# Zehong-Ma/OVMR

Measured on AMD Instinct MI355X. Metric: images/sec ViT-B/16 encode+fusion, 1k-class×16-shot, 1/2/4/8 MI355X, higher is better.
Workload: dtype f16; 1 GPU; OVMR classifier generation + fusion inference, ViT-B/16, 1000 classes x 16 shots (16000 exemplar images, batch 775) + 4096 query images (batch 256), n_ctx 2, tau 10; parallelism=class/query sharding over 1 rank(s); all-gather rows + all-reduce counters, preset=metric, gemm_variant=8, attn_variant=3, ln_fold=1, gelu_exact=0, stream_text=1, encoder_reserve_images=775, encoder_chunk_images=775, output_dir=tmpfs scratch (/dev/shm)

## Files before the change

### ovmr_amd/csrc/common.h

```cpp
#pragma once
#include <hip/hip_runtime.h>
#include <stdint.h>

typedef _Float16 half_t;
typedef _Float16 half2_t __attribute__((ext_vector_type(2)));
typedef _Float16 half4_t __attribute__((ext_vector_type(4)));
typedef _Float16 half8_t __attribute__((ext_vector_type(8)));
typedef float float4_t __attribute__((ext_vector_type(4)));
typedef float float2_t __attribute__((ext_vector_type(2)));

#define OVMR_WAVE 64
#define OVMR_MAX_DEVICES 64

enum {
    EPI_NONE = 0,
    EPI_BIAS = 1,
    EPI_BIAS_QGELU = 2,
    EPI_BIAS_RES = 3,
    EPI_PATCH = 4,
    EPI_SCALE = 5,
    EPI_LN_BIAS = 6,
    EPI_LN_BIAS_QGELU = 7,
    EPI_SCALE_ARGMAX = 8,
};

struct GemmArgs {
    const void* A; int lda;
    const void* W; int ldw;
    void* C; int ldc;
    const void* bias;
    const void* res; int ldres;
    const void* pos;
    int M, N, K;
    int epi;
    int rows_in, rows_out;
    float scale;
    int n_group;
    const float* ln_stats; int ln_slots;
    int ln_stride;
    const float* ln_g; const float* ln_b;
    float* stats_out;
    int nt_store;
    float* argmax_out;
    int gelu_mode;
    int im2col_R;
};

__device__ __forceinline__ float quick_gelu_h(float u) {
    half_t t = (half_t)(1.702f * u);
    half_t s = (half_t)__builtin_amdgcn_rcpf(1.0f + __builtin_amdgcn_exp2f(-1.4426950408889634f * (float)t));
    return (float)(half_t)(u * (float)s);
}

__device__ __forceinline__ half4_t quick_gelu_h4(half4_t u) {
    half4_t t;
    float4_t e;
#pragma unroll
    for (int k = 0; k < 4; ++k) {
        t[k] = (half_t)(1.702f * (float)u[k]);
        e[k] = __builtin_amdgcn_exp2f(fminf(__builtin_fmaf((float)t[k], -1.4426950408889634f, 0.0f), 30.0f));
    }
    const float2_t p = (float2_t){e[0], e[2]} + 1.0f, q = (float2_t){e[1], e[3]} + 1.0f;
    const float2_t pq = p * q;
    const float R = __builtin_amdgcn_rcpf(pq[0] * pq[1]);
    const float2_t rr = (float2_t){pq[1], pq[0]} * R;
// ... 46 lines not shown
```

### ovmr_amd/csrc/gemm_f16.hip

```cpp
#include "gemm_epi.h"
#include "gemm_route.h"

namespace {

constexpr int BK = 64;

template <int EPI>
__global__ __launch_bounds__(256) void gemm_f16_t128(GemmArgs a) {
    extern __shared__ __attribute__((aligned(16))) char smem[];
    half_t* sA = (half_t*)smem;
    half_t* sB = sA + 2 * 128 * BK;

    const int tid = threadIdx.x, lane = tid & 63, wave = tid >> 6;
    const int wm = wave >> 1, wn = wave & 1;
    const int tiles_n = (a.N + 127) >> 7;
    const int tm = blockIdx.x / tiles_n, tn = blockIdx.x - tm * tiles_n;
    const int m0 = tm << 7, n0 = tn << 7;

    const half_t* A = (const half_t*)a.A;
    const half_t* W = (const half_t*)a.W;

    const int lc = tid & 7, lr = tid >> 3;
    const int sw = ((lc ^ (lr & 7)) << 3);
    const half_t* ga[4];
// ... 81 lines not shown
        HIP_CHECK_RET(hipFuncSetAttribute((const void*)gemm_f16_t128<EPI>, hipFuncAttributeMaxDynamicSharedMemorySize, (int)lds));
        attr_set[dev] = true;
    }
    hipLaunchKernelGGL(gemm_f16_t128<EPI>, dim3(tiles), dim3(256), lds, s, a);
    return (int)hipGetLastError();
}

bool one_round_of_s64(int M, int N) { return (long)((M + 63) / 64) * ((N + 63) / 64) <= 256; }
bool aligned16(const void* p) { return ((uintptr_t)p & 15) == 0; }

void plan_tile(const GemmArgs& a, bool ping_pong, GemmPlan& p) {
    const int tiles_n = (a.N + 255) / 256;
    const double t256 = (double)((a.M + 255) / 256) * tiles_n, t128 = (double)((a.M + 127) / 128) * tiles_n;
    auto rounds = [](double t) { return ceil(t / 256.0); };
    auto eff = [&](double t) { return t / (rounds(t) * 256.0); };
    const bool big = ping_pong ? rounds(t256) <= 0.74 * rounds(t128) : t256 >= 64 && eff(t256) + 0.08 >= eff(t128);
    p.tile_rows = big ? 256 : 128;
    const int tiles = (int)(big ? t256 : t128);
    const bool res = a.epi == EPI_BIAS_RES, lnf = a.epi == EPI_LN_BIAS || a.epi == EPI_LN_BIAS_QGELU;
    p.loop = ping_pong && big ? LOOP_PINGPONG : (lnf || (res && a.K >= 2048)) ? LOOP_BOUNDARY : LOOP_DOUBLE;
    p.a_nt = res && tiles_n <= 4 && tiles >= 512;
    p.nt_store = !res && a.epi != EPI_SCALE_ARGMAX && (size_t)a.M * a.N * 2 >= ((size_t)48 << 20);
    p.n_group = p.loop == LOOP_PINGPONG && tiles_n >= 8 ? 4 : tiles_n;
}

}

bool gemm_f16_latency_bound(int variant, int M, int N) { return variant == 8 && one_round_of_s64(M, N); }
int gemm_f16_pinned_variant(int variant, int M, int N) { return variant != 8 ? variant : one_round_of_s64(M, N) ? 9 : 7; }

GemmPlan gemm_f16_route(const GemmArgs& a, int variant) {
    GemmPlan p = {};
    auto run = [&p](int kernel, int rc = 0) { p.kernel = kernel; p.rc = rc; return p; };
    auto none = [&run](int rc) { return run(GEMM_NONE, rc); };
    const bool lnf = a.epi == EPI_LN_BIAS || a.epi == EPI_LN_BIAS_QGELU, res = a.epi == EPI_BIAS_RES, argmax = a.epi == EPI_SCALE_ARGMAX;
    if (a.epi == EPI_BIAS_QGELU || a.epi == EPI_LN_BIAS_QGELU) p.gelu_mode = variant >= 100 ? variant / 100 : a.gelu_mode;
    if (variant >= 100) variant %= 100;
    if (a.M <= 0 || a.N <= 0) return none(0);
    if (a.K <= 0 || (a.K % BK) != 0 || (a.lda & 7) || (a.ldw & 7)) return none(-2);
    const bool tile_only = a.im2col_R || argmax || lnf || a.stats_out;
    if (!tile_only && (variant == 9 || gemm_f16_latency_bound(variant, a.M, a.N)) && (a.K % 128) == 0 && aligned16(a.A) && aligned16(a.W) && a.epi != EPI_PATCH &&
        a.epi >= EPI_NONE && a.epi <= EPI_SCALE) {
        const int steps = a.K >> 7, tiles = ((a.M + 63) >> 6) * ((a.N + 63) >> 6);
        p.depth = steps % 4 == 0 && tiles <= 256 ? 4 : steps % 3 == 0 ? 3 : steps % 2 == 0 ? 2 : 1;
        p.groups = steps / p.depth;
        return run(GEMM_S64);
// ... 1 lines not shown
    const bool takes = a.M >= 256 && a.N >= 128 && (long)a.M * a.lda * 2 < 0x7fffffffL && (long)a.N * a.ldw * 2 < 0x7fffffffL &&
                       (argmax ? a.argmax_out != nullptr
                               : !(a.N & 7) && !(a.ldc & 7) && aligned16(a.C) && (!res || (!(a.ldres & 7) && aligned16(a.res))));
    if ((tile_only || variant >= 1) && takes) {
        if (a.im2col_R) {
            const int G = a.im2col_R >> 4;
            if (a.epi != EPI_PATCH || a.K != 768 || (a.im2col_R & 15) || a.rows_in != G * G || !aligned16(a.A) ||
                (long)((a.M + a.rows_in - 1) / a.rows_in) * 3 * a.im2col_R * a.im2col_R * 2 >= 0x7fffffffL)
                return none(-2);
        }
        if (lnf && ((a.N & 63) || !a.ln_stats || a.ln_slots < 1 || !a.ln_g || !a.ln_b)) return none(-2);
        if (a.stats_out && (!res || (a.N & 255))) return none(-2);
        const int loop = (variant == 0 || variant == 7 || variant == 9) ? 8 : variant;
        if (loop != 6 && loop != 8) return none(-5);
        if (a.epi < EPI_NONE || a.epi > EPI_SCALE_ARGMAX) return none(-3);
        plan_tile(a, loop == 8 && (a.K % 128) == 0, p);
        return run(GEMM_TILE);
    }
    if (tile_only) return none(-4);
    if (a.epi < EPI_NONE || a.epi > EPI_SCALE) return none(-3);
    return run(GEMM_T128);
}

extern "C" int ovmr_debug_gemm_route(int variant, int M, int N, int K, int epi, int ldc, int ldres, int stats, int im2col, int* out) {
    static float operand[4];
    alignas(16) static char base[16];
    GemmArgs a = {};
    a.M = M; a.N = N; a.K = a.lda = a.ldw = K; a.epi = epi; a.ldc = ldc; a.ldres = ldres;
    a.A = a.W = a.res = base; a.C = base;
    a.ln_stats = a.ln_g = a.ln_b = operand; a.ln_slots = 1; a.argmax_out = operand; a.stats_out = stats ? operand : nullptr;
    a.im2col_R = im2col; a.rows_in = (im2col >> 4) * (im2col >> 4); a.rows_out = a.rows_in + 1;
    static_assert(sizeof(GemmPlan) == 10 * sizeof(int), "");
    *(GemmPlan*)out = gemm_f16_route(a, variant);
    return 0;
}

int launch_gemm_f16(const GemmArgs& a_in, int variant, hipStream_t s) {
    const GemmPlan p = gemm_f16_route(a_in, variant);
    GemmArgs a = a_in;
    a.n_group = p.n_group;
    a.gelu_mode = p.gelu_mode;
    switch (p.kernel) {
        case GEMM_T128:
#define X(E) if (a.epi == E) return launch_t128<E>(a, s);
            X(EPI_NONE) X(EPI_BIAS) X(EPI_BIAS_QGELU) X(EPI_BIAS_RES) X(EPI_PATCH) X(EPI_SCALE)
#undef X
            return -3;
        case GEMM_S64: return launch_gemm_f16_small(a, p, s);
        case GEMM_TILE: return launch_gemm_f16_v5(a, p, s);
    }
    return p.rc;
}
```

### ovmr_amd/csrc/gemm_f16_v5.hip

```cpp
#include "gemm_route.h"

namespace {

constexpr int BK5 = 64, BN5 = 256;
typedef const __attribute__((address_space(1))) void* gptr_t;
typedef __attribute__((address_space(3))) void* lptr_t;

template <int CTRL>
__device__ __forceinline__ float dpp_f32(float v) {
    return __builtin_bit_cast(float, __builtin_amdgcn_update_dpp(0, __builtin_bit_cast(int, v), CTRL, 0xF, 0xF, true));
}

constexpr int OPT_A_NT = 1;
constexpr int OPT_BOUNDARY = 4;
constexpr int OPT_PINGPONG = 16;
constexpr int OPT_NT_STORE = 512;
constexpr int OPT_GELU_F32 = 2048;
template <int EPI, int MT, int OPT>
__global__ __launch_bounds__(512) void gemm_f16_v5_kernel(GemmArgs a, int tiles_m, int tiles_n) {
    constexpr int BM = MT * 32;
    constexpr int A_BYTES = BM * 128, STAGE = (BM + BN5) * 128;
    constexpr int AJ = BM / 64;
    constexpr bool NT = OPT & OPT_NT_STORE;
    constexpr int EP = 128;
    constexpr bool GFAST = (OPT & OPT_GELU_F32) != 0;
    constexpr bool LNF = EPI == EPI_LN_BIAS || EPI == EPI_LN_BIAS_QGELU;
    constexpr bool HAS_BIAS = EPI == EPI_BIAS || EPI == EPI_BIAS_QGELU || EPI == EPI_BIAS_RES;
    extern __shared__ __attribute__((aligned(16))) char smem[];
    float* col_c = (float*)(smem + 2 * STAGE);
    float* row_c = col_c + 2 * BN5;

    const int tid = threadIdx.x, lane = tid & 63;
    const int wave = __builtin_amdgcn_readfirstlane(tid >> 6);
    const int wm = wave >> 2, wn = wave & 3;

    const int nwg = tiles_m * tiles_n;
    int bid = blockIdx.x;
    {
        const int xcd = bid & 7, idx = bid >> 3, q = nwg >> 3, r = nwg & 7;
        bid = (xcd < r ? xcd * (q + 1) : r * (q + 1) + (xcd - r) * q) + idx;
    }
    int tm, tn;
    {
        const int G = a.n_group > 0 ? a.n_group : tiles_n;
        const int full = tiles_n / G, per = tiles_m * G;
        const int g = bid / per;
        if (g < full) {
            const int r = bid - g * per;
            tm = r / G;
            tn = g * G + (r - tm * G);
        } else {
            const int Gl = tiles_n - full * G, r = bid - full * per;
            tm = r / Gl;
            tn = full * G + (r - tm * Gl);
        }
    }
    const int m0 = tm * BM, n0 = tn * BN5;

    const int nk = a.K / BK5;
    const half_t* A = (const half_t*)a.A;
    const half_t* W = (const half_t*)a.W;

    const int srow = lane >> 3, slot = lane & 7;
    const int schunk = (slot ^ srow) * 8;
    unsigned oa[AJ], ob[4];
    auto src_off = [&](int row, int ld) -> unsigned { return (unsigned)(((long)row * ld + schunk) * 2); };
    const int imR = (EPI == EPI_PATCH) ? a.im2col_R : 0;
    auto a_off = [&](int row) -> unsigned {
        if (EPI == EPI_PATCH && imR) {
            const int G = imR >> 4, r = min(row, a.M - 1), b = r / a.rows_in, p = r - b * a.rows_in, gy = p / G, gx = p - gy * G;
            const int c8 = schunk >> 3;
            return (unsigned)(2 * (((long)b * 3 * imR + gy * 16 + (c8 >> 1)) * imR + gx * 16 + (c8 & 1) * 8));
        }
        return src_off(min(row, a.M - 1), a.lda);
    };
    auto a_tile = [&](int kt) -> const char* {
        if (EPI == EPI_PATCH && imR) return (const char*)A + 2 * ((long)(kt >> 2) * imR * imR + (kt & 3) * 4 * imR);
        return (const char*)A + (long)kt * 128;
    };
#pragma unroll
// ... 9 lines not shown
    const int ldsA_w = wave * (BM / 8) * 128;
    const int ldsB_w = A_BYTES + wave * 32 * 128;

    auto stage = [&](int buf, int kt) {
        char* base = smem + buf * STAGE;
#pragma unroll
        for (int j = 0; j < AJ; ++j)
            __builtin_amdgcn_global_load_lds((gptr_t)(a_tile(kt) + oa[j]), (lptr_t)(base + ldsA_w + j * 1024), 16, 0, (OPT & OPT_A_NT) ? 2 : 0);
#pragma unroll
        for (int j = 0; j < 4; ++j)
            __builtin_amdgcn_global_load_lds((gptr_t)((const char*)W + ob[j] + (long)kt * 128), (lptr_t)(base + ldsB_w + j * 1024), 16, 0, 0);
    };

    float4_t acc[MT][4];
#pragma unroll
    for (int i = 0; i < MT; ++i)
#pragma unroll
        for (int j = 0; j < 4; ++j) acc[i][j] = (float4_t){0.f, 0.f, 0.f, 0.f};

    const int fr = lane & 15, fg = lane >> 4;
    const int a_row_off = (wm * (BM / 2) + fr) * 128;
    const int b_row_off = A_BYTES + (wn * 64 + fr) * 128;
    const int ch0 = ((fg) ^ (fr & 7)) << 4, ch1 = ((4 + fg) ^ (fr & 7)) << 4;

    constexpr bool PH8 = (OPT & OPT_PINGPONG) != 0 && MT == 8;
    if (!PH8) stage(0, 0);

    if (PH8) {
    } else if (tid < BN5) {
        const int n = n0 + tid;
        float c0 = 0.f, c1 = 0.f;
        if (n < a.N) {
            if (HAS_BIAS) c0 = (float)((const half_t*)a.bias)[n];
            if (LNF) { c0 = a.ln_g[n]; c1 = a.ln_b[n]; }
        }
        col_c[tid] = c0;
        col_c[BN5 + tid] = c1;
    } else if (LNF && tid - BN5 < BM) {
        const int r = tid - BN5;
        const float2_t* sp = (const float2_t*)a.ln_stats + (long)min(m0 + r, a.M - 1) * (a.ln_stride ? a.ln_stride : a.ln_slots);
        float su = 0.f, sq = 0.f;
        for (int sl = 0; sl < a.ln_slots; ++sl) { const float2_t p = sp[sl]; su += p[0]; sq += p[1]; }
        const float inv_k = 1.0f / (float)a.K;
        const float mean = su * inv_k;
        const float rstd = 1.0f / sqrtf(fmaxf(sq * inv_k - mean * mean, 0.f) + 1e-5f);
        row_c[r] = rstd;
        row_c[BM + r] = -rstd * mean;
    }

    if constexpr (PH8) {
    constexpr int SLOT = 16384, KBUF = 4 * SLOT;
    enum { hB0 = 0, hA0 = 1, hB1 = 2, hA1 = 3 };
    unsigned sa8[2][2], sb8[2][2];
#pragma unroll
    for (int hf = 0; hf < 2; ++hf)
#pragma unroll
        for (int j = 0; j < 2; ++j) {
            const int lr = wave * 16 + j * 8 + srow;
            const int ra = m0 + (lr >> 6) * 128 + hf * 64 + (lr & 63);
            const int rb = n0 + (lr >> 5) * 64 + hf * 32 + (lr & 31);
            sa8[hf][j] = a_off(ra);
            sb8[hf][j] = src_off(min(rb, a.N - 1), a.ldw);
        }
    const unsigned smem_lds = __builtin_amdgcn_readfirstlane((unsigned)(uintptr_t)(lptr_t)smem);
    const unsigned wave_lds = (unsigned)__builtin_amdgcn_readfirstlane(wave * 2048);
    auto stage_half = [&](int buf, int which, int kt) {
        const int hf = which >> 1;
        const char* ak = a_tile(kt);
        const char* wk = (const char*)W + (long)kt * 128;
#pragma unroll
        for (int j = 0; j < 2; ++j) {
            const unsigned dst = smem_lds + (unsigned)(buf * KBUF + which * SLOT + j * 1024) + wave_lds;
            if (which & 1) {
                if constexpr ((OPT & OPT_A_NT) != 0) asm volatile("s_mov_b32 m0, %2\n\ts_nop 0\n\tglobal_load_lds_dwordx4 %0, %1 nt" :: "v"(sa8[hf][j]), "s"(ak), "s"(dst) : "memory", "m0");
                else asm volatile("s_mov_b32 m0, %2\n\ts_nop 0\n\tglobal_load_lds_dwordx4 %0, %1" :: "v"(sa8[hf][j]), "s"(ak), "s"(dst) : "memory", "m0");
            } else {
                asm volatile("s_mov_b32 m0, %2\n\ts_nop 0\n\tglobal_load_lds_dwordx4 %0, %1" :: "v"(sb8[hf][j]), "s"(wk), "s"(dst) : "memory", "m0");
            }
        }
    };
    const int a_lane = (wm * 64 + fr) * 128, b_lane = (wn * 32 + fr) * 128;
    half8_t fa[4][2], fb0[2][2], fb1[2][2];
    auto read_a = [&](const char* buf, int hf) {
#pragma unroll
        for (int ii = 0; ii < 4; ++ii) {
            fa[ii][0] = *(const half8_t*)(buf + (1 + 2 * hf) * SLOT + a_lane + ii * 2048 + ch0);
// ... 2 lines not shown
    };
    auto read_b = [&](const char* buf, int g, half8_t (&fb)[2][2]) {
#pragma unroll
        for (int jj = 0; jj < 2; ++jj) {
            fb[jj][0] = *(const half8_t*)(buf + 2 * g * SLOT + b_lane + jj * 2048 + ch0);
            fb[jj][1] = *(const half8_t*)(buf + 2 * g * SLOT + b_lane + jj * 2048 + ch1);
        }
    };
    auto quadrant = [&](int hf, int g, half8_t (&fb)[2][2]) {
        __builtin_amdgcn_s_setprio(1);
#pragma unroll
        for (int st = 0; st < 2; ++st)
#pragma unroll
            for (int ii = 0; ii < 4; ++ii)
#pragma unroll
                for (int jj = 0; jj < 2; ++jj)
                    acc[hf * 4 + ii][g * 2 + jj] = __builtin_amdgcn_mfma_f32_16x16x32_f16(fb[jj][st], fa[ii][st], acc[hf * 4 + ii][g * 2 + jj], 0, 0, 0);
        __builtin_amdgcn_s_setprio(0);
    };
#define OVMR_PH_END()                                                     \
    __builtin_amdgcn_sched_barrier(0);                                    \
    __builtin_amdgcn_s_barrier();                                         \
    __builtin_amdgcn_sched_barrier(0);
    stage_half(0, hB0, 0); stage_half(0, hA0, 0); stage_half(0, hB1, 0); stage_half(0, hA1, 0);
    if (tid < BN5) {
        const int n = n0 + tid;
        float c0 = 0.f, c1 = 0.f;
        if (n < a.N) {
            if (HAS_BIAS) c0 = (float)((const half_t*)a.bias)[n];
            if (LNF) { c0 = a.ln_g[n]; c1 = a.ln_b[n]; }
        }
        col_c[tid] = c0;
        col_c[BN5 + tid] = c1;
    } else if (LNF && tid - BN5 < BM) {
        const int r = tid - BN5;
        const float2_t* sp = (const float2_t*)a.ln_stats + (long)min(m0 + r, a.M - 1) * (a.ln_stride ? a.ln_stride : a.ln_slots);
        float su = 0.f, sq = 0.f;
        for (int sl = 0; sl < a.ln_slots; ++sl) { const float2_t p = sp[sl]; su += p[0]; sq += p[1]; }
        const float inv_k = 1.0f / (float)a.K;
        const float mean = su * inv_k;
        const float rstd = 1.0f / sqrtf(fmaxf(sq * inv_k - mean * mean, 0.f) + 1e-5f);
        row_c[r] = rstd;
        row_c[BM + r] = -rstd * mean;
    }
    __builtin_amdgcn_sched_barrier(0);
    stage_half(1, hB0, 1); stage_half(1, hA0, 1);
    asm volatile("s_waitcnt vmcnt(4)" ::: "memory");
    asm volatile("s_waitcnt lgkmcnt(0)" ::: "memory");
    __builtin_amdgcn_s_barrier();
    __builtin_amdgcn_sched_barrier(0);
    if (wm == 1) __builtin_amdgcn_s_barrier();
    __builtin_amdgcn_sched_barrier(0);
    const char* const bufE = smem;
    const char* const bufO = smem + KBUF;
#define OVMR_P4_MID()                                                     \
    __builtin_amdgcn_sched_barrier(0);                                    \
    asm volatile("s_waitcnt lgkmcnt(0)" ::: "memory");                    \
    __builtin_amdgcn_s_barrier();                                         \
    __builtin_amdgcn_sched_barrier(0);
    for (int kt = 0; kt < nk; kt += 2) {
        const bool more = kt + 2 < nk;
        read_b(bufE, 0, fb0);
        read_a(bufE, 0);
        read_b(bufE, 1, fb1);
        __builtin_amdgcn_sched_barrier(0);
        stage_half(1, hB1, kt + 1); stage_half(1, hA1, kt + 1);
        OVMR_P4_MID()
        quadrant(0, 0, fb0);
        quadrant(0, 1, fb1);
// ... 10 lines not shown
        OVMR_PH_END()
        read_b(bufO, 0, fb0);
        read_a(bufO, 0);
        read_b(bufO, 1, fb1);
        __builtin_amdgcn_sched_barrier(0);
        if (more) { stage_half(0, hB1, kt + 2); stage_half(0, hA1, kt + 2); }
        OVMR_P4_MID()
        quadrant(0, 0, fb0);
        quadrant(0, 1, fb1);
        OVMR_PH_END()
        read_a(bufO, 1);
        __builtin_amdgcn_sched_barrier(0);
        if (more) { stage_half(1, hB0, kt + 3); stage_half(1, hA0, kt + 3); }
        __builtin_amdgcn_sched_barrier(0);
        if (more) asm volatile("s_waitcnt vmcnt(4)" ::: "memory");
        OVMR_P4_MID()
        quadrant(1, 1, fb1);
        quadrant(1, 0, fb0);
        OVMR_PH_END()
    }
#undef OVMR_P4_MID
    if (wm == 0) __builtin_amdgcn_s_barrier();
    __builtin_amdgcn_sched_barrier(0);
#undef OVMR_PH_END
    } else
    if (OPT & OPT_BOUNDARY) {
    constexpr int D = 2, R = D + 2;
    static_assert((2 * MT) % R == 0 && D <= MT, "");
    half8_t fb[2][4], fa[R];
    auto first_reads = [&](const char* buf) {
#pragma unroll
        for (int t = 0; t < 4; ++t) fb[0][t] = *(const half8_t*)(buf + b_row_off + t * 2048 + ch0);
#pragma unroll
        for (int t = 0; t < D; ++t) fa[t] = *(const half8_t*)(buf + a_row_off + (t % MT) * 2048 + (t / MT ? ch1 : ch0));
    };
    asm volatile("s_waitcnt vmcnt(0)" ::: "memory");
    asm volatile("s_waitcnt lgkmcnt(0)" ::: "memory");
    __builtin_amdgcn_s_barrier();
    __builtin_amdgcn_sched_barrier(0);
    first_reads(smem);
    __builtin_amdgcn_sched_barrier(0);
    if (nk > 1) stage(1, 1);
    __builtin_amdgcn_sched_barrier(0);
    for (int kt = 0; kt < nk; ++kt) {
        const char* cur = smem + (kt & 1) * STAGE;
#pragma unroll
// ... 109 lines not shown
                int* d = arg_lds + ((wm * (BM / 2) + i * 16 + fr) * 4 + wn) * 2;
                d[0] = __float_as_int(bv);
                d[1] = bc;
            }
        }
        __syncthreads();
        if (tid < BM && m0 + tid < a.M) {
            float bv = __int_as_float(arg_lds[tid * 8]);
            int bc = arg_lds[tid * 8 + 1];
#pragma unroll
            for (int w = 1; w < 4; ++w) {
                const float v = __int_as_float(arg_lds[tid * 8 + 2 * w]);
                const int vc = arg_lds[tid * 8 + 2 * w + 1];
                if (v > bv || (v == bv && vc < bc)) { bv = v; bc = vc; }
            }
            int* dst = (int*)a.argmax_out + ((long)(m0 + tid) * tiles_n + tn) * 2;
            dst[0] = __float_as_int(bv);
            dst[1] = bc;
        }
        return;
    }
    char* et = smem + wave * (64 * EP);
    const int er = lane >> 3, ec = (lane & 7) * 8;
    const int fsw = ((fr & 7) << 1) | (fr >> 3);
    int wr_off[4];
#pragma unroll
    for (int j = 0; j < 4; ++j) wr_off[j] = fr * EP + (((j * 4 + fg) ^ fsw) << 3);
    const int rd_off = er * EP + (((lane & 7) ^ er) << 4);
    auto read_staged = [&](int it) -> half8_t {
        const half8_t v = *(const half8_t*)(et + it * 8 * EP + rd_off);
        if (it & 1) return (half8_t){v[4], v[5], v[6], v[7], v[0], v[1], v[2], v[3]};
        return v;
    };
    const bool emit_stats = EPI == EPI_BIAS_RES && a.stats_out != nullptr;
    const bool full_tile = EPI != EPI_PATCH && m0 + BM <= a.M && n0 + BN5 <= a.N;
    float* stat_lds = (float*)(smem + 8 * 64 * EP);
#pragma unroll
    for (int h = 0; h < MT / 4; ++h) {
        if (h == 0) __syncthreads();
        half8_t res8[EPI == EPI_BIAS_RES ? 8 : 1];
        if (EPI == EPI_BIAS_RES) {
            const int nn = n0 + wn * 64 + ec;
#pragma unroll
            for (int it = 0; it < 8; ++it) {
                const int m = min(m0 + wm * (BM / 2) + h * 64 + it * 8 + er, a.M - 1);
                res8[EPI == EPI_BIAS_RES ? it : 0] = *(const half8_t*)((const half_t*)a.res + (long)m * a.ldres + min(nn, a.N - 8));
            }
        }
        float ln_rs[LNF ? 4 : 1], ln_ts[LNF ? 4 : 1];
        if (LNF) {
#pragma unroll
            for (int i = 0; i < 4; ++i) {
                const int r = wm * (BM / 2) + h * 64 + i * 16 + fr;
                ln_rs[LNF ? i : 0] = row_c[r];
                ln_ts[LNF ? i : 0] = row_c[BM + r];
            }
        }
#pragma unroll
        for (int j = 0; j < 4; ++j) {
            const int cc = wn * 64 + j * 16 + fg * 4;
            const float4_t c0 = *(const float4_t*)(col_c + cc);
            float4_t c1 = c0;
            if (LNF) c1 = *(const float4_t*)(col_c + BN5 + cc);
#pragma unroll
            for (int i = 0; i < 4; ++i) {
                const float4_t v = acc[h * 4 + i][j];
                const float ln_r = ln_rs[LNF ? i : 0], ln_t = ln_ts[LNF ? i : 0];
                half4_t o;
                if (LNF) {
#pragma unroll
                    for (int r = 0; r < 4; r += 2) {
                        const float2_t t2 = __builtin_elementwise_fma((float2_t){ln_t, ln_t}, (float2_t){c0[r], c0[r + 1]}, (float2_t){c1[r], c1[r + 1]});
                        float2_t x2 = __builtin_elementwise_fma((float2_t){ln_r, ln_r}, (float2_t){v[r], v[r + 1]}, t2);
                        if (EPI == EPI_LN_BIAS_QGELU && GFAST) x2 = quick_gelu_f32x2(x2);
                        const half2_t u2 = __builtin_convertvector(x2, half2_t);
                        o[r] = u2[0];
                        o[r + 1] = u2[1];
                    }
                    if (EPI == EPI_LN_BIAS_QGELU && !GFAST) o = quick_gelu_h4(o);
                } else {
#pragma unroll
                    for (int r = 0; r < 4; r += 2) {
                        float2_t x2 = {v[r], v[r + 1]};
                        if (HAS_BIAS) x2 += (float2_t){c0[r], c0[r + 1]};
                        if (EPI == EPI_BIAS_QGELU && GFAST) x2 = quick_gelu_f32x2(x2);
                        half2_t u2 = __builtin_convertvector(x2, half2_t);
                        if (EPI == EPI_SCALE) {
                            float2_t y2 = __builtin_convertvector(u2, float2_t);
                            y2 *= a.scale;
                            u2 = __builtin_convertvector(y2, half2_t);
                        }
                        o[r] = u2[0];
                        o[r + 1] = u2[1];
                    }
                    if (EPI == EPI_BIAS_QGELU && !GFAST) o = quick_gelu_h4(o);
                }
                *(half4_t*)(et + i * 16 * EP + wr_off[j]) = o;
            }
        }
        const int nn = n0 + wn * 64 + ec;
        auto finish = [&](half8_t v, int it, int row) -> half8_t {
            if (EPI == EPI_BIAS_RES) {
// ... 45 lines not shown
#pragma unroll
                        for (int k = 0; k < 8; ++k) v[k] = (half_t)((float)v[k] + (float)p8[k]);
                    }
                    half8_t* dst = (half8_t*)(C + crow * a.ldc + nn);
                    if (NT) __builtin_nontemporal_store(v, dst);
                    else *dst = v;
                }
            }
        }
    }
    if (emit_stats) {
        asm volatile("s_waitcnt lgkmcnt(0)" ::: "memory");
        __builtin_amdgcn_s_barrier();
        asm volatile("" ::: "memory");
        if (tid < BM && m0 + tid < a.M) {
            const float* p = stat_lds + tid * 8;
            const float su = ((p[0] + p[2]) + p[4]) + p[6], sq = ((p[1] + p[3]) + p[5]) + p[7];
            *(float2_t*)(a.stats_out + ((long)(m0 + tid) * tiles_n + tn) * 2) = (float2_t){su, sq};
        }
    }
}

template <int EPI, int MT, int OPT>
int launch_v5_k(const GemmArgs& b, int tiles_m, int tiles_n, hipStream_t s) {
    constexpr int BM = MT * 32;
    const size_t lds = (size_t)2 * (BM + BN5) * 128 + 2 * BN5 * 4 + 2 * BM * 4;
    static bool attr_set[OVMR_MAX_DEVICES] = {};
    int dev = 0;
    HIP_CHECK_RET(hipGetDevice(&dev));
    if (dev >= 0 && dev < OVMR_MAX_DEVICES && !attr_set[dev]) {
        HIP_CHECK_RET(hipFuncSetAttribute((const void*)gemm_f16_v5_kernel<EPI, MT, OPT>, hipFuncAttributeMaxDynamicSharedMemorySize, (int)lds));
        attr_set[dev] = true;
    }
    hipLaunchKernelGGL((gemm_f16_v5_kernel<EPI, MT, OPT>), dim3(tiles_m * tiles_n), dim3(512), lds, s, b, tiles_m, tiles_n);
    return (int)hipGetLastError();
}

#define V5_DOUBLE_PP(X, E, F) X(E, 4, (F)) X(E, 8, (F)) X(E, 8, (F) | OPT_PINGPONG)
#define V5_BOUNDARY(X, E, F) X(E, 4, (F) | OPT_BOUNDARY) X(E, 8, (F) | OPT_BOUNDARY)
#define V5_STORES(X, LOOPS, E, F) LOOPS(X, E, (F)) LOOPS(X, E, (F) | OPT_NT_STORE)
#define V5_BOUNDARY_PP(X, E, F) V5_BOUNDARY(X, E, F) X(E, 8, (F) | OPT_PINGPONG)
#define V5_TABLE(X)                                                                                                                \
    V5_STORES(X, V5_DOUBLE_PP, EPI_NONE, 0) V5_STORES(X, V5_DOUBLE_PP, EPI_BIAS, 0)                                                 \
    V5_STORES(X, V5_DOUBLE_PP, EPI_PATCH, 0) V5_STORES(X, V5_DOUBLE_PP, EPI_SCALE, 0)                                               \
    V5_STORES(X, V5_DOUBLE_PP, EPI_BIAS_QGELU, 0) V5_STORES(X, V5_DOUBLE_PP, EPI_BIAS_QGELU, OPT_GELU_F32)                          \
    V5_DOUBLE_PP(X, EPI_BIAS_RES, 0) V5_DOUBLE_PP(X, EPI_BIAS_RES, OPT_A_NT) V5_BOUNDARY(X, EPI_BIAS_RES, 0) V5_BOUNDARY(X, EPI_BIAS_RES, OPT_A_NT) \
    V5_STORES(X, V5_BOUNDARY_PP, EPI_LN_BIAS, 0) V5_DOUBLE_PP(X, EPI_SCALE_ARGMAX, 0)                                               \
    V5_STORES(X, V5_BOUNDARY_PP, EPI_LN_BIAS_QGELU, 0) V5_STORES(X, V5_BOUNDARY_PP, EPI_LN_BIAS_QGELU, OPT_GELU_F32)

}

int launch_gemm_f16_v5(const GemmArgs& a, const GemmPlan& p, hipStream_t s) {
    const int mt = p.tile_rows / 32, tiles_m = (a.M + p.tile_rows - 1) / p.tile_rows, tiles_n = (a.N + BN5 - 1) / BN5;
    const int opt = (p.a_nt ? OPT_A_NT : 0) | (p.loop == LOOP_BOUNDARY ? OPT_BOUNDARY : 0) | (p.loop == LOOP_PINGPONG ? OPT_PINGPONG : 0) |
                    (p.nt_store ? OPT_NT_STORE : 0) | (p.gelu_mode ? OPT_GELU_F32 : 0);
#define X(E, MT, OPT) if (a.epi == E && mt == MT && opt == (OPT)) return launch_v5_k<E, MT, (OPT)>(a, tiles_m, tiles_n, s);
    V5_TABLE(X)
#undef X
    return -3;
}

extern "C" int ovmr_debug_gemm_tile_kernels(int* out, int cap) {
    int n = 0;
#define X(E, MT, OPT) if (n < cap) { out[3 * n] = E; out[3 * n + 1] = MT; out[3 * n + 2] = (OPT); } ++n;
    V5_TABLE(X)
#undef X
    return n;
}
```

### ovmr_amd/csrc/gemm_route.h

```cpp
#pragma once
#include "common.h"

enum GemmKernel {
    GEMM_NONE = 0,
    GEMM_T128 = 1,
    GEMM_S64 = 2,
    GEMM_TILE = 3,
};
enum GemmLoop { LOOP_DOUBLE = 0, LOOP_BOUNDARY = 1, LOOP_PINGPONG = 2 };

struct GemmPlan {
    int kernel, rc;
    int depth, groups;
    int tile_rows, loop, a_nt, nt_store, n_group;
    int gelu_mode;
};
GemmPlan gemm_f16_route(const GemmArgs& a, int variant);
int launch_gemm_f16_small(const GemmArgs& a, const GemmPlan& p, hipStream_t s);
int launch_gemm_f16_v5(const GemmArgs& a, const GemmPlan& p, hipStream_t s);
bool gemm_f16_latency_bound(int variant, int M, int N);
int gemm_f16_pinned_variant(int variant, int M, int N);
```

### ovmr_amd/csrc/ovmr_api.hip

```cpp
#include "../../include/ovmr_hip.h"
#include "carver.h"
#include "gemm_route.h"

#include <algorithm>
#include <array>
#include <cmath>
#include <cstdarg>
#include <cstdio>
#include <cstdlib>
#include <cstring>
#include <map>
#include <string>
#include <vector>

namespace {

struct Buf {
    void* p = nullptr;
    size_t elems = 0;
    int f32 = 0;
    std::vector<int64_t> shape;
};

struct Block {
    void *in_w, *in_b, *out_w, *out_b, *fc_w, *fc_b, *pj_w, *pj_b;
    float *ln1_g, *ln1_b, *ln2_g, *ln2_b;
    half_t *in_wf = nullptr, *fc_wf = nullptr;
    float *in_g = nullptr, *in_bf = nullptr, *fc_g = nullptr, *fc_bf = nullptr;
};

}

struct ovmr_handle {
    ovmr_model_desc d;
    std::map<std::string, Buf> w;
    std::vector<void*> owned;
    std::vector<void*> derived;
    std::string err;
    bool finalized = false;
    int gelu_exact = 0;
    int last_q_cls = 1;
    int fuse_im2col = 1;
    int gemm_variant = 8, attn_variant = 3;
    int ln_fold = 1;
    int xval_fused = 1;
    int fused_head = 1;
    int head_max_grid = 0;
    int* head_sync = nullptr;
    float logit_scale_exp = 100.f;
    bool have_logit_scale = false;

    std::vector<Block> vis, txt, agg;
    half_t *conv_w = nullptr, *pos16_vis = nullptr, *cls_pos16 = nullptr, *proj_t = nullptr;
    half_t *pos16_txt = nullptr, *textproj_t = nullptr;
    void *conv1 = nullptr, *cls_emb = nullptr, *pos_vis = nullptr, *proj = nullptr, *pos_txt = nullptr, *textproj = nullptr;
    float *ln_pre_g = nullptr, *ln_pre_b = nullptr, *ln_post_g = nullptr, *ln_post_b = nullptr;
    float *ln_final_g = nullptr, *ln_final_b = nullptr, *tok_emb = nullptr, *cls_token = nullptr;
    int Kpad = 0, G = 0, L = 0;

    char* ws = nullptr;
    size_t ws_bytes = 0;
    int max_images = 0, max_prompts = 0, max_classes = 0;
    int enc_chunk_forced = 0;
    int n_cu = 0;
    int enc_chunk = 0;
    int enc_fold = 0;
    int img_cap = 0;
// ... 160 lines not shown
            rc = OVMR_E_NOMEM;
        if (!rc) rc = launch_fold_ln((const half_t*)W, gamma, beta, (const half_t*)bias, wf, g, bf, N, K, s);
    }
    ~LnFoldScratch() {
        (void)hipStreamSynchronize(s);
        (void)hipFree(stats); (void)hipFree(g); (void)hipFree(bf); (void)hipFree(wf);
    }
};

struct LnLinear { const float *ln_g, *ln_b; const half_t *w, *b, *wf; const float *g, *bf; bool gelu; };
LnLinear in_proj(const Block& k) { return {k.ln1_g, k.ln1_b, (const half_t*)k.in_w, (const half_t*)k.in_b, k.in_wf, k.in_g, k.in_bf, false}; }
LnLinear c_fc(const Block& k) { return {k.ln2_g, k.ln2_b, (const half_t*)k.fc_w, (const half_t*)k.fc_b, k.fc_wf, k.fc_g, k.fc_bf, true}; }

struct LnPart { int r0, n, M, step; half_t* C; int ldc; };

int ln_linear(ovmr_handle* h, const LnLinear& l, const half_t* x, half_t* y, int rows, int W, const float* stats, int variant,
              std::initializer_list<LnPart> parts, hipStream_t s) {
    if (!stats) CK(launch_layernorm(x, y, l.ln_g, l.ln_b, rows, W, W, 0, s));
    const int slots = W / 256, epi = l.gelu ? (stats ? EPI_LN_BIAS_QGELU : EPI_BIAS_QGELU) : (stats ? EPI_LN_BIAS : EPI_BIAS);
    for (const LnPart& p : parts) {
        GemmArgs a = gemm(stats ? x : y, p.step * W, (stats ? l.wf : l.w) + (size_t)p.r0 * W, W, p.C, p.ldc, p.M, p.n, W, epi, stats ? nullptr : l.b + p.r0);
        if (stats) { a = gemm_ln(a, stats, slots, l.g + p.r0, l.bf + p.r0); a.ln_stride = p.step * slots; }
        a.gelu_mode = l.gelu && !h->gelu_exact;
        CK(launch_gemm_f16(a, variant, s));
    }
    return 0;
}

struct SeqGroup { int nseq, L; long row0; };

int run_block_f16(ovmr_handle* h, const Block& k, half_t* x, half_t* y, half_t* qkv, half_t* hid,
                  int nseq, int L, int W, int causal, hipStream_t s, float* stats = nullptr,
                  const std::vector<SeqGroup>* groups = nullptr, half_t* cls_rows = nullptr) {
    int M = nseq * L;
    if (groups) { M = 0; for (auto& g : *groups) M += g.nseq * g.L; }
    const int H = W / 64;
    if (cls_rows && nseq >= 256 && h->last_q_cls) {
        CK(ln_linear(h, in_proj(k), x, y, M, W, stats, gemm_f16_pinned_variant(h->gemm_variant, M, 3 * W),
                     {{W, 2 * W, M, 1, qkv + W, 3 * W}, {0, W, nseq, L, qkv, L * 3 * W}}, s));
    } else
        CK(ln_linear(h, in_proj(k), x, y, M, W, stats, h->gemm_variant, {{0, 3 * W, M, 1, qkv, 3 * W}}, s));
    if (cls_rows)
        CK(launch_attention_f16_q(qkv, y, nseq, L, 1, H, causal, h->attn_variant, s));
    else if (groups) {
        int rc = -100;
        if (h->attn_variant >= 1 && groups->size() <= 4) {
// ... 224 lines not shown
        const int left = B - b0 - Bc;
        if (left > 0 && left <= h->enc_fold && Bc + left <= h->img_cap) Bc += left;
        plan.push_back(Bc);
        b0 += Bc;
    }
    return plan;
}

int ovmr_set_option(ovmr_handle* h, const char* key, int value) {
    if (!h || !key) return OVMR_E_ARG;
    if (!strcmp(key, "gemm")) h->gemm_variant = value;
    else if (!strcmp(key, "attn")) h->attn_variant = value;
    else if (!strcmp(key, "fuse_im2col")) h->fuse_im2col = value != 0;
    else if (!strcmp(key, "last_q_cls")) h->last_q_cls = value != 0;
    else if (!strcmp(key, "enc_chunk")) {
        h->enc_chunk_forced = value > 0 ? value : 0;
        if (h->finalized) set_enc_chunk(h);
    }
    else if (!strcmp(key, "ln_fold")) h->ln_fold = value;
    else if (!strcmp(key, "xval_fused")) h->xval_fused = value;
    else if (!strcmp(key, "fused_head")) h->fused_head = value;
    else if (!strcmp(key, "head_max_grid")) h->head_max_grid = value;
    else if (!strcmp(key, "gelu_exact")) h->gelu_exact = value;
    else if (!strcmp(key, "agg_max_len")) {
        if (value < 128 || value > OVMR_AGG_MAX_LEN_CEILING)
            return fail(h, OVMR_E_ARG, "agg_max_len %d outside [128,%d]", value, OVMR_AGG_MAX_LEN_CEILING);
        h->agg_max_len = value;
    }
    else return fail(h, OVMR_E_NAME, "unknown option '%s'", key);
    return 0;
}

float ovmr_logit_scale(const ovmr_handle* h) { return h ? h->logit_scale_exp : 0.f; }

int ovmr_preprocess_u8(const void* u8_hwc, int B, int R, const float* mean3, const float* std3, void* out_f16, ovmr_stream stream) {
    if (B == 0) return 0;
    if (!u8_hwc || !out_f16 || !mean3 || !std3 || B < 0 || R <= 0) return OVMR_E_ARG;
    if (R % 8) return OVMR_E_SHAPE;
    return launch_preprocess_u8((const uint8_t*)u8_hwc, (half_t*)out_f16, B, R, mean3, std3, (hipStream_t)stream);
}

int ovmr_resize_crop_u8(const void* pixels, const ovmr_resize_job* jobs, int n, const int32_t* tables, void* tmp, int max_ny,
                        void* out_u8, int R, ovmr_stream stream) {
    if (n == 0) return 0;
    if (!pixels || !jobs || !tables || !out_u8 || n < 0 || R <= 0 || max_ny < 0 || (max_ny > 0 && !tmp)) return OVMR_E_ARG;
    return launch_resize_crop_u8((const uint8_t*)pixels, jobs, n, tables, (uint8_t*)tmp, max_ny, (uint8_t*)out_u8, R, (hipStream_t)stream);
// ... 599 lines not shown
```

Baseline: 29840 images/s.

## Make LN-folded ping-pong GEMM persistent with overlapped next-tile prefetch

For LayerNorm-folded GEMMs using the 256-row ping-pong loop with more than 256 tiles, the kernel now launches one workgroup per CU and loops over tiles. It prefetches the next tile's K-slices and LN constants while running the current tile's epilogue, and double-buffers the constants in LDS. The aim is to hide per-tile prologue and epilogue latency and avoid tail waves. The cost is more LDS per workgroup, lower occupancy, and a more complex control flow; it is enabled by default behind a gemm_persist option.

```diff
diff --git a/ovmr_amd/csrc/common.h b/ovmr_amd/csrc/common.h
--- a/ovmr_amd/csrc/common.h
+++ b/ovmr_amd/csrc/common.h
@@ -40,7 +40,7 @@
     int ln_stride;
     const float* ln_g; const float* ln_b;
     float* stats_out;
-    int nt_store;
+    int persist;
     float* argmax_out;
     int gelu_mode;
     int im2col_R;
diff --git a/ovmr_amd/csrc/gemm_f16.hip b/ovmr_amd/csrc/gemm_f16.hip
--- a/ovmr_amd/csrc/gemm_f16.hip
+++ b/ovmr_amd/csrc/gemm_f16.hip
@@ -1,3 +1,5 @@
+#include <string.h>
+
 #include "gemm_epi.h"
 #include "gemm_route.h"
 
@@ -127,6 +129,7 @@
     p.a_nt = res && tiles_n <= 4 && tiles >= 512;
     p.nt_store = !res && a.epi != EPI_SCALE_ARGMAX && (size_t)a.M * a.N * 2 >= ((size_t)48 << 20);
     p.n_group = p.loop == LOOP_PINGPONG && tiles_n >= 8 ? 4 : tiles_n;
+    p.persist = a.persist && lnf && p.loop == LOOP_PINGPONG && tiles > 256;
 }
 
 }
@@ -174,7 +177,7 @@
     return run(GEMM_T128);
 }
 
-extern "C" int ovmr_debug_gemm_route(int variant, int M, int N, int K, int epi, int ldc, int ldres, int stats, int im2col, int* out) {
+extern "C" int ovmr_debug_gemm_plan(int variant, int M, int N, int K, int epi, int ldc, int ldres, int stats, int im2col, int persist, int* out) {
     static float operand[4];
     alignas(16) static char base[16];
     GemmArgs a = {};
@@ -182,9 +185,37 @@
     a.A = a.W = a.res = base; a.C = base;
     a.ln_stats = a.ln_g = a.ln_b = operand; a.ln_slots = 1; a.argmax_out = operand; a.stats_out = stats ? operand : nullptr;
     a.im2col_R = im2col; a.rows_in = (im2col >> 4) * (im2col >> 4); a.rows_out = a.rows_in + 1;
-    static_assert(sizeof(GemmPlan) == 10 * sizeof(int), "");
+    a.persist = persist;
+    static_assert(sizeof(GemmPlan) == 11 * sizeof(int), "");
     *(GemmPlan*)out = gemm_f16_route(a, variant);
     return 0;
+}
+
+extern "C" int ovmr_debug_gemm_route(int variant, int M, int N, int K, int epi, int ldc, int ldres, int stats, int im2col, int* out) {
+    int plan[11];
+    const int rc = ovmr_debug_gemm_plan(variant, M, N, K, epi, ldc, ldres, stats, im2col, 0, plan);
+    memcpy(out, plan, 10 * sizeof(int));
+    return rc;
+}
+
+extern "C" int ovmr_debug_gemm_persist(int variant, const void* A, int lda, const void* W, const float* ln_b, const float* ln_stats, int ln_slots,
+                                       int ln_stride, const float* ln_g, void* C, int ldc, int M, int N, int K, int epi, int persist, int max_wgs,
+                                       void* stream) {
+    if (epi != EPI_LN_BIAS && epi != EPI_LN_BIAS_QGELU) return -1;
+    if (!A || !W || !ln_b || !ln_stats || !ln_g || !C || max_wgs < 0) return -1;
+    GemmArgs a = {};
+    a.A = A; a.lda = lda; a.W = W; a.ldw = K; a.C = C; a.ldc = ldc; a.M = M; a.N = N; a.K = K; a.epi = epi; a.scale = 1.f;
+    a.ln_stats = ln_stats; a.ln_slots = ln_slots; a.ln_stride = ln_stride; a.ln_g = ln_g; a.ln_b = ln_b;
+    a.persist = persist;
+    if (!max_wgs) return launch_gemm_f16(a, variant, (hipStream_t)stream);
+    GemmPlan p = gemm_f16_route(a, variant);
+    if (p.kernel != GEMM_TILE) return p.kernel == GEMM_NONE ? p.rc : -4;
+    if (K % 128) return -2;
+    const int tiles_n = (N + 255) / 256;
+    p.tile_rows = 256; p.loop = LOOP_PINGPONG; p.a_nt = 0; p.n_group = tiles_n >= 8 ? 4 : tiles_n; p.persist = 1;
+    a.n_group = p.n_group;
+    a.gelu_mode = p.gelu_mode;
+    return launch_gemm_f16_v5(a, p, (hipStream_t)stream, max_wgs);
 }
 
 int launch_gemm_f16(const GemmArgs& a_in, int variant, hipStream_t s) {
diff --git a/ovmr_amd/csrc/gemm_f16_v5.hip b/ovmr_amd/csrc/gemm_f16_v5.hip
--- a/ovmr_amd/csrc/gemm_f16_v5.hip
+++ b/ovmr_amd/csrc/gemm_f16_v5.hip
@@ -1,3 +1,6 @@
+#include <algorithm>
+#include <type_traits>
+
 #include "gemm_route.h"
 
 namespace {
@@ -16,6 +19,30 @@
 constexpr int OPT_PINGPONG = 16;
 constexpr int OPT_NT_STORE = 512;
 constexpr int OPT_GELU_F32 = 2048;
+
+constexpr bool v5_tile_loop(int epi, int mt, int opt) { return (epi == EPI_LN_BIAS || epi == EPI_LN_BIAS_QGELU) && mt == 8 && (opt & OPT_PINGPONG); }
+constexpr int V5_CONST_BLOCK = 4096, V5_STAGING = 16384;
+
+__host__ __device__ __forceinline__ void v5_tile_of(int bid, int tiles_m, int tiles_n, int n_group, int& tm, int& tn) {
+    const int nwg = tiles_m * tiles_n;
+    {
+        const int xcd = bid & 7, idx = bid >> 3, q = nwg >> 3, r = nwg & 7;
+        bid = (xcd < r ? xcd * (q + 1) : r * (q + 1) + (xcd - r) * q) + idx;
+    }
+    const int G = n_group > 0 ? n_group : tiles_n;
+    const int full = tiles_n / G, per = tiles_m * G;
+    const int g = bid / per;
+    if (g < full) {
+        const int r = bid - g * per;
+        tm = r / G;
+        tn = g * G + (r - tm * G);
+    } else {
+        const int Gl = tiles_n - full * G, r = bid - full * per;
+        tm = r / Gl;
+        tn = full * G + (r - tm * Gl);
+    }
+}
+
 template <int EPI, int MT, int OPT>
 __global__ __launch_bounds__(512) void gemm_f16_v5_kernel(GemmArgs a, int tiles_m, int tiles_n) {
     constexpr int BM = MT * 32;
@@ -34,28 +61,10 @@
     const int wave = __builtin_amdgcn_readfirstlane(tid >> 6);
     const int wm = wave >> 2, wn = wave & 3;
 
-    const int nwg = tiles_m * tiles_n;
-    int bid = blockIdx.x;
-    {
-        const int xcd = bid & 7, idx = bid >> 3, q = nwg >> 3, r = nwg & 7;
-        bid = (xcd < r ? xcd * (q + 1) : r * (q + 1) + (xcd - r) * q) + idx;
-    }
+    constexpr bool LOOPED = v5_tile_loop(EPI, MT, OPT);
     int tm, tn;
-    {
-        const int G = a.n_group > 0 ? a.n_group : tiles_n;
-        const int full = tiles_n / G, per = tiles_m * G;
-        const int g = bid / per;
-        if (g < full) {
-            const int r = bid - g * per;
-            tm = r / G;
-            tn = g * G + (r - tm * G);
-        } else {
-            const int Gl = tiles_n - full * G, r = bid - full * per;
-            tm = r / Gl;
-            tn = full * G + (r - tm * Gl);
-        }
-    }
-    const int m0 = tm * BM, n0 = tn * BN5;
+    v5_tile_of(blockIdx.x, tiles_m, tiles_n, a.n_group, tm, tn);
+    int m0 = tm * BM, n0 = tn * BN5;
 
     const int nk = a.K / BK5;
     const half_t* A = (const half_t*)a.A;
@@ -111,6 +120,27 @@
     const int a_row_off = (wm * (BM / 2) + fr) * 128;
     const int b_row_off = A_BYTES + (wn * 64 + fr) * 128;
     const int ch0 = ((fg) ^ (fr & 7)) << 4, ch1 = ((4 + fg) ^ (fr & 7)) << 4;
+
+    auto ln_fold4 = [&](const float4_t v, const float ln_r, const float ln_t, const float4_t c0, const float4_t c1) -> half4_t {
+        half4_t o;
+#pragma unroll
+        for (int r = 0; r < 4; r += 2) {
+            const float2_t t2 = __builtin_elementwise_fma((float2_t){ln_t, ln_t}, (float2_t){c0[r], c0[r + 1]}, (float2_t){c1[r], c1[r + 1]});
+            float2_t x2 = __builtin_elementwise_fma((float2_t){ln_r, ln_r}, (float2_t){v[r], v[r + 1]}, t2);
+            if (EPI == EPI_LN_BIAS_QGELU && GFAST) x2 = quick_gelu_f32x2(x2);
+            const half2_t u2 = __builtin_convertvector(x2, half2_t);
+            o[r] = u2[0];
+            o[r + 1] = u2[1];
+        }
+        if (EPI == EPI_LN_BIAS_QGELU && !GFAST) o = quick_gelu_h4(o);
+        return o;
+    };
+    auto stage_wr = [&](int j) -> int { return fr * EP + (((j * 4 + fg) ^ (((fr & 7) << 1) | (fr >> 3))) << 3); };
+    auto stage_rd = [&]() -> int { return (lane >> 3) * EP + (((lane & 7) ^ (lane >> 3)) << 4); };
+    auto stage_unswap = [](const half8_t v, int it) -> half8_t {
+        if (it & 1) return (half8_t){v[4], v[5], v[6], v[7], v[0], v[1], v[2], v[3]};
+        return v;
+    };
 
     constexpr bool PH8 = (OPT & OPT_PINGPONG) != 0 && MT == 8;
     if (!PH8) stage(0, 0);
@@ -141,16 +171,19 @@
     constexpr int SLOT = 16384, KBUF = 4 * SLOT;
     enum { hB0 = 0, hA0 = 1, hB1 = 2, hA1 = 3 };
     unsigned sa8[2][2], sb8[2][2];
-#pragma unroll
-    for (int hf = 0; hf < 2; ++hf)
-#pragma unroll
-        for (int j = 0; j < 2; ++j) {
-            const int lr = wave * 16 + j * 8 + srow;
-            const int ra = m0 + (lr >> 6) * 128 + hf * 64 + (lr & 63);
-            const int rb = n0 + (lr >> 5) * 64 + hf * 32 + (lr & 31);
-            sa8[hf][j] = a_off(ra);
-            sb8[hf][j] = src_off(min(rb, a.N - 1), a.ldw);
-        }
+    auto source_rows = [&](int tm0, int tn0) {
+#pragma unroll
+        for (int hf = 0; hf < 2; ++hf)
+#pragma unroll
+            for (int j = 0; j < 2; ++j) {
+                const int lr = wave * 16 + j * 8 + srow;
+                const int ra = tm0 + (lr >> 6) * 128 + hf * 64 + (lr & 63);
+                const int rb = tn0 + (lr >> 5) * 64 + hf * 32 + (lr & 31);
+                sa8[hf][j] = a_off(ra);
+                sb8[hf][j] = src_off(min(rb, a.N - 1), a.ldw);
+            }
+    };
+    source_rows(m0, n0);
     const unsigned smem_lds = __builtin_amdgcn_readfirstlane((unsigned)(uintptr_t)(lptr_t)smem);
     const unsigned wave_lds = (unsigned)__builtin_amdgcn_readfirstlane(wave * 2048);
     auto stage_half = [&](int buf, int which, int kt) {
@@ -199,7 +232,45 @@
     __builtin_amdgcn_sched_barrier(0);                                    \
     __builtin_amdgcn_s_barrier();                                         \
     __builtin_amdgcn_sched_barrier(0);
+    float cr[8];
+    auto load_consts = [&](int tm0, int tn0) {
+#pragma unroll
+        for (int q = 0; q < 8; ++q) cr[q] = 0.f;
+        if (tid < BN5) {
+            const int n = tn0 + tid;
+            if (n < a.N) { cr[0] = a.ln_g[n]; cr[1] = a.ln_b[n]; }
+        } else {
+            const float2_t* sp = (const float2_t*)a.ln_stats + (long)min(tm0 + tid - BN5, a.M - 1) * (a.ln_stride ? a.ln_stride : a.ln_slots);
+#pragma unroll
+            for (int sl = 0; sl < 4; ++sl)
+                if (sl < a.ln_slots) { const float2_t p = sp[sl]; cr[2 * sl] = p[0]; cr[2 * sl + 1] = p[1]; }
+        }
+    };
+    auto store_consts = [&](int blk, int tm0) {
+        float* cc = (float*)(smem + 2 * KBUF + blk * V5_CONST_BLOCK);
+        if (tid < BN5) {
+            cc[tid] = cr[0];
+            cc[BN5 + tid] = cr[1];
+        } else {
+            const int r = tid - BN5;
+            const float2_t* sp = (const float2_t*)a.ln_stats + (long)min(tm0 + r, a.M - 1) * (a.ln_stride ? a.ln_stride : a.ln_slots);
+            float su = 0.f, sq = 0.f;
+#pragma unroll
+            for (int sl = 0; sl < 4; ++sl)
+                if (sl < a.ln_slots) { su += cr[2 * sl]; sq += cr[2 * sl + 1]; }
+            for (int sl = 4; sl < a.ln_slots; ++sl) { const float2_t p = sp[sl]; su += p[0]; sq += p[1]; }
+            const float inv_k = 1.0f / (float)a.K;
+            const float mean = su * inv_k;
+            const float rstd = 1.0f / sqrtf(fmaxf(sq * inv_k - mean * mean, 0.f) + 1e-5f);
+            cc[2 * BN5 + r] = rstd;
+            cc[2 * BN5 + BM + r] = -rstd * mean;
+        }
+    };
     stage_half(0, hB0, 0); stage_half(0, hA0, 0); stage_half(0, hB1, 0); stage_half(0, hA1, 0);
+    if constexpr (LOOPED) {
+        load_consts(m0, n0);
+        store_consts(0, m0);
+    } else
     if (tid < BN5) {
         const int n = n0 + tid;
         float c0 = 0.f, c1 = 0.f;
@@ -222,6 +293,7 @@
     }
     __builtin_amdgcn_sched_barrier(0);
     stage_half(1, hB0, 1); stage_half(1, hA0, 1);
+    for (int dslot = blockIdx.x, cb = 0;; cb ^= 1) {
     asm volatile("s_waitcnt vmcnt(4)" ::: "memory");
     asm volatile("s_waitcnt lgkmcnt(0)" ::: "memory");
     __builtin_amdgcn_s_barrier();
@@ -278,6 +350,66 @@
 #undef OVMR_P4_MID
     if (wm == 0) __builtin_amdgcn_s_barrier();
     __builtin_amdgcn_sched_barrier(0);
+    if constexpr (!LOOPED) break;
+    else {
+        const int cm0 = m0, cn0 = n0;
+        dslot += (int)gridDim.x;
+        const bool next = dslot < tiles_m * tiles_n;
+        if (next) {
+            v5_tile_of(dslot, tiles_m, tiles_n, a.n_group, tm, tn);
+            m0 = tm * BM;
+            n0 = tn * BN5;
+            source_rows(m0, n0);
+            load_consts(m0, n0);
+            __builtin_amdgcn_sched_barrier(0);
+            stage_half(0, hB0, 0); stage_half(0, hA0, 0); stage_half(0, hB1, 0); stage_half(0, hA1, 0);
+            stage_half(1, hB0, 1); stage_half(1, hA0, 1);
+            __builtin_amdgcn_sched_barrier(0);
+        }
+        half_t* const C = (half_t*)a.C;
+        const float* const ccol = (const float*)(smem + 2 * KBUF + cb * V5_CONST_BLOCK);
+        const float* const crow = ccol + 2 * BN5;
+        char* const et = smem + 2 * KBUF + 2 * V5_CONST_BLOCK + wave * (16 * EP);
+        const int er = lane >> 3, nn = cn0 + wn * 64 + (lane & 7) * 8;
+        const int rd_off = stage_rd();
+        const bool full_tile = cm0 + BM <= a.M && cn0 + BN5 <= a.N;
+        float4_t c0[4], c1[4];
+#pragma unroll
+        for (int j = 0; j < 4; ++j) {
+            c0[j] = *(const float4_t*)(ccol + wn * 64 + j * 16 + fg * 4);
+            c1[j] = *(const float4_t*)(ccol + BN5 + wn * 64 + j * 16 + fg * 4);
+        }
+        auto convert_and_store = [&](auto guarded) {
+            half_t* dst = C + (long)(cm0 + wm * (BM / 2) + er) * a.ldc + nn;
+            const long step = 8L * a.ldc;
+#pragma unroll
+            for (int i = 0; i < MT; ++i) {
+                const int r = wm * (BM / 2) + i * 16 + fr;
+                const float ln_r = crow[r], ln_t = crow[BM + r];
+#pragma unroll
+                for (int j = 0; j < 4; ++j) *(half4_t*)(et + stage_wr(j)) = ln_fold4(acc[i][j], ln_r, ln_t, c0[j], c1[j]);
+                half8_t vv[2];
+#pragma unroll
+                for (int it = 0; it < 2; ++it) vv[it] = stage_unswap(*(const half8_t*)(et + it * 8 * EP + rd_off), it);
+#pragma unroll
+                for (int it = 0; it < 2; ++it, dst += step) {
+                    if (decltype(guarded)::value && !(cm0 + wm * (BM / 2) + i * 16 + it * 8 + er < a.M && nn < a.N)) continue;
+                    if (NT) __builtin_nontemporal_store(vv[it], (half8_t*)dst);
+                    else *(half8_t*)dst = vv[it];
+                }
+                __builtin_amdgcn_sched_barrier(0);
+            }
+            if (next) store_consts(cb ^ 1, m0);
+        };
+        if (full_tile) convert_and_store(std::false_type{});
+        else convert_and_store(std::true_type{});
+        if (!next) return;
+#pragma unroll
+        for (int i = 0; i < MT; ++i)
+#pragma unroll
+            for (int j = 0; j < 4; ++j) acc[i][j] = (float4_t){0.f, 0.f, 0.f, 0.f};
+    }
+    }
 #undef OVMR_PH_END
     } else
     if (OPT & OPT_BOUNDARY) {
@@ -433,15 +565,12 @@
     }
     char* et = smem + wave * (64 * EP);
     const int er = lane >> 3, ec = (lane & 7) * 8;
-    const int fsw = ((fr & 7) << 1) | (fr >> 3);
     int wr_off[4];
 #pragma unroll
-    for (int j = 0; j < 4; ++j) wr_off[j] = fr * EP + (((j * 4 + fg) ^ fsw) << 3);
-    const int rd_off = er * EP + (((lane & 7) ^ er) << 4);
+    for (int j = 0; j < 4; ++j) wr_off[j] = stage_wr(j);
+    const int rd_off = stage_rd();
     auto read_staged = [&](int it) -> half8_t {
-        const half8_t v = *(const half8_t*)(et + it * 8 * EP + rd_off);
-        if (it & 1) return (half8_t){v[4], v[5], v[6], v[7], v[0], v[1], v[2], v[3]};
-        return v;
+        return stage_unswap(*(const half8_t*)(et + it * 8 * EP + rd_off), it);
     };
     const bool emit_stats = EPI == EPI_BIAS_RES && a.stats_out != nullptr;
     const bool full_tile = EPI != EPI_PATCH && m0 + BM <= a.M && n0 + BN5 <= a.N;
@@ -479,16 +608,7 @@
                 const float ln_r = ln_rs[LNF ? i : 0], ln_t = ln_ts[LNF ? i : 0];
                 half4_t o;
                 if (LNF) {
-#pragma unroll
-                    for (int r = 0; r < 4; r += 2) {
-                        const float2_t t2 = __builtin_elementwise_fma((float2_t){ln_t, ln_t}, (float2_t){c0[r], c0[r + 1]}, (float2_t){c1[r], c1[r + 1]});
-                        float2_t x2 = __builtin_elementwise_fma((float2_t){ln_r, ln_r}, (float2_t){v[r], v[r + 1]}, t2);
-                        if (EPI == EPI_LN_BIAS_QGELU && GFAST) x2 = quick_gelu_f32x2(x2);
-                        const half2_t u2 = __builtin_convertvector(x2, half2_t);
-                        o[r] = u2[0];
-                        o[r + 1] = u2[1];
-                    }
-                    if (EPI == EPI_LN_BIAS_QGELU && !GFAST) o = quick_gelu_h4(o);
+                    o = ln_fold4(v, ln_r, ln_t, c0, c1);
                 } else {
 #pragma unroll
                     for (int r = 0; r < 4; r += 2) {
@@ -580,9 +700,11 @@
 }
 
 template <int EPI, int MT, int OPT>
-int launch_v5_k(const GemmArgs& b, int tiles_m, int tiles_n, hipStream_t s) {
+int launch_v5_k(const GemmArgs& b, int tiles_m, int tiles_n, int max_wgs, hipStream_t s) {
     constexpr int BM = MT * 32;
-    const size_t lds = (size_t)2 * (BM + BN5) * 128 + 2 * BN5 * 4 + 2 * BM * 4;
+    constexpr bool LOOPED = v5_tile_loop(EPI, MT, OPT);
+    const size_t lds = LOOPED ? (size_t)2 * (BM + BN5) * 128 + 2 * V5_CONST_BLOCK + V5_STAGING : (size_t)2 * (BM + BN5) * 128 + 2 * BN5 * 4 + 2 * BM * 4;
+    static_assert(2 * BN5 * 4 + 2 * 256 * 4 == V5_CONST_BLOCK && 8 * 16 * 128 == V5_STAGING, "");
     static bool attr_set[OVMR_MAX_DEVICES] = {};
     int dev = 0;
     HIP_CHECK_RET(hipGetDevice(&dev));
@@ -590,7 +712,8 @@
         HIP_CHECK_RET(hipFuncSetAttribute((const void*)gemm_f16_v5_kernel<EPI, MT, OPT>, hipFuncAttributeMaxDynamicSharedMemorySize, (int)lds));
         attr_set[dev] = true;
     }
-    hipLaunchKernelGGL((gemm_f16_v5_kernel<EPI, MT, OPT>), dim3(tiles_m * tiles_n), dim3(512), lds, s, b, tiles_m, tiles_n);
+    const int tiles = tiles_m * tiles_n, grid = LOOPED && max_wgs > 0 ? std::min(tiles, max_wgs) : tiles;
+    hipLaunchKernelGGL((gemm_f16_v5_kernel<EPI, MT, OPT>), dim3(grid), dim3(512), lds, s, b, tiles_m, tiles_n);
     return (int)hipGetLastError();
 }
 
@@ -608,14 +731,36 @@
 
 }
 
-int launch_gemm_f16_v5(const GemmArgs& a, const GemmPlan& p, hipStream_t s) {
+int launch_gemm_f16_v5(const GemmArgs& a, const GemmPlan& p, hipStream_t s, int max_wgs) {
     const int mt = p.tile_rows / 32, tiles_m = (a.M + p.tile_rows - 1) / p.tile_rows, tiles_n = (a.N + BN5 - 1) / BN5;
     const int opt = (p.a_nt ? OPT_A_NT : 0) | (p.loop == LOOP_BOUNDARY ? OPT_BOUNDARY : 0) | (p.loop == LOOP_PINGPONG ? OPT_PINGPONG : 0) |
                     (p.nt_store ? OPT_NT_STORE : 0) | (p.gelu_mode ? OPT_GELU_F32 : 0);
-#define X(E, MT, OPT) if (a.epi == E && mt == MT && opt == (OPT)) return launch_v5_k<E, MT, (OPT)>(a, tiles_m, tiles_n, s);
+    int wgs = 0;
+    if (p.persist) {
+        static int n_cu[OVMR_MAX_DEVICES] = {};
+        int dev = 0;
+        HIP_CHECK_RET(hipGetDevice(&dev));
+        if (dev < 0 || dev >= OVMR_MAX_DEVICES) return -100;
+        if (!n_cu[dev]) HIP_CHECK_RET(hipDeviceGetAttribute(&n_cu[dev], hipDeviceAttributeMultiprocessorCount, dev));
+        wgs = std::max(1, n_cu[dev]);
+        if (max_wgs > 0) wgs = std::min(wgs, max_wgs);
+    }
+#define X(E, MT, OPT) if (a.epi == E && mt == MT && opt == (OPT)) return launch_v5_k<E, MT, (OPT)>(a, tiles_m, tiles_n, wgs, s);
     V5_TABLE(X)
 #undef X
     return -3;
+}
+
+extern "C" int ovmr_debug_gemm_tile_walk(int tiles_m, int tiles_n, int n_group, int grid, int* out, int cap) {
+    if (tiles_m < 1 || tiles_n < 1 || grid < 1 || !out) return -1;
+    int n = 0;
+    for (int w = 0; w < grid; ++w)
+        for (int slot = w; slot < tiles_m * tiles_n; slot += grid, ++n)
+            if (n < cap) {
+                out[3 * n] = w;
+                v5_tile_of(slot, tiles_m, tiles_n, n_group, out[3 * n + 1], out[3 * n + 2]);
+            }
+    return n;
 }
 
 extern "C" int ovmr_debug_gemm_tile_kernels(int* out, int cap) {
diff --git a/ovmr_amd/csrc/gemm_route.h b/ovmr_amd/csrc/gemm_route.h
--- a/ovmr_amd/csrc/gemm_route.h
+++ b/ovmr_amd/csrc/gemm_route.h
@@ -14,9 +14,10 @@
     int depth, groups;
     int tile_rows, loop, a_nt, nt_store, n_group;
     int gelu_mode;
+    int persist;
 };
 GemmPlan gemm_f16_route(const GemmArgs& a, int variant);
 int launch_gemm_f16_small(const GemmArgs& a, const GemmPlan& p, hipStream_t s);
-int launch_gemm_f16_v5(const GemmArgs& a, const GemmPlan& p, hipStream_t s);
+int launch_gemm_f16_v5(const GemmArgs& a, const GemmPlan& p, hipStream_t s, int max_wgs = 0);
 bool gemm_f16_latency_bound(int variant, int M, int N);
 int gemm_f16_pinned_variant(int variant, int M, int N);
diff --git a/ovmr_amd/csrc/ovmr_api.hip b/ovmr_amd/csrc/ovmr_api.hip
--- a/ovmr_amd/csrc/ovmr_api.hip
+++ b/ovmr_amd/csrc/ovmr_api.hip
@@ -43,6 +43,7 @@
     int fuse_im2col = 1;
     int gemm_variant = 8, attn_variant = 3;
     int ln_fold = 1;
+    int gemm_persist = 1;
     int xval_fused = 1;
     int fused_head = 1;
     int head_max_grid = 0;
@@ -249,6 +250,7 @@
         GemmArgs a = gemm(stats ? x : y, p.step * W, (stats ? l.wf : l.w) + (size_t)p.r0 * W, W, p.C, p.ldc, p.M, p.n, W, epi, stats ? nullptr : l.b + p.r0);
         if (stats) { a = gemm_ln(a, stats, slots, l.g + p.r0, l.bf + p.r0); a.ln_stride = p.step * slots; }
         a.gelu_mode = l.gelu && !h->gelu_exact;
+        a.persist = h->gemm_persist;
         CK(launch_gemm_f16(a, variant, s));
     }
     return 0;
@@ -519,6 +521,7 @@
     else if (!strcmp(key, "fused_head")) h->fused_head = value;
     else if (!strcmp(key, "head_max_grid")) h->head_max_grid = value;
     else if (!strcmp(key, "gelu_exact")) h->gelu_exact = value;
+    else if (!strcmp(key, "gemm_persist")) h->gemm_persist = value != 0;
     else if (!strcmp(key, "agg_max_len")) {
         if (value < 128 || value > OVMR_AGG_MAX_LEN_CEILING)
             return fail(h, OVMR_E_ARG, "agg_max_len %d outside [128,%d]", value, OVMR_AGG_MAX_LEN_CEILING);
```

After: 30470 images/s (median of 6 runs). 2.1% higher.
